# omahs/cess

Hardware: AMD Instinct MI355X
Metric: verified BLS12-381 sigs/sec (node) (higher is better)
Workload: dtype u32 (381-bit Montgomery, 14x28-bit limb products via v_mad_u64_u32)

## Files before the change

cess_amd/csrc/bls/consts.hpp:

```cpp
#pragma once
#include <stdint.h>
#ifndef CESS_CONST
#define CESS_CONST static constexpr
#endif
namespace bls { namespace c {
CESS_CONST uint32_t P_RAW[12] = {0xffffaaabu, 0xb9feffffu, 0xb153ffffu, 0x1eabfffeu, 0xf6b0f624u, 0x6730d2a0u, 0xf38512bfu, 0x64774b84u, 0x434bacd7u, 0x4b1ba7b6u, 0x397fe69au, 0x1a0111eau};
CESS_CONST uint32_t P2_RAW[12] = {0xffff5556u, 0x73fdffffu, 0x62a7ffffu, 0x3d57fffdu, 0xed61ec48u, 0xce61a541u, 0xe70a257eu, 0xc8ee9709u, 0x869759aeu, 0x96374f6cu, 0x72ffcd34u, 0x340223d4u};
CESS_CONST uint32_t ONE[12] = {0x0347fcb8u, 0x19d80000u, 0x6d2002b1u, 0x12e00cdeu, 0xa2090c72u, 0x37669f83u, 0xda0f73e0u, 0x09b09b42u, 0x8f1297bbu, 0xa7c515d9u, 0xfcfa012cu, 0x0577a659u};
CESS_CONST uint32_t R2[12] = {0x510370edu, 0x626d1c34u, 0xc53e243du, 0xd65aec45u, 0x3317d3b1u, 0x4f36a009u, 0x5d74088bu, 0x8c10ea72u, 0x75865d11u, 0xd507320au, 0xa759fd5cu, 0x0c8d4cc8u};
CESS_CONST uint32_t R2_384[12] = {0xc4d1dd0eu, 0x9941d94cu, 0x51c109f3u, 0xff568cb5u, 0x0df0c2b7u, 0x1cc8ea98u, 0x76862c67u, 0xdbf76e0cu, 0x47ae37e1u, 0xcef527bfu, 0x56b3b194u, 0x0834704du};
CESS_CONST uint32_t P28[14] = {0xfffaaabu, 0xfefffffu, 0x3ffffb9u, 0xfffeb15u, 0x6241eabu, 0xa0f6b0fu, 0xf6730d2u, 0xf38512bu, 0x4774b84u, 0x4bacd76u, 0xba7b643u, 0xe69a4b1u, 0x1ea397fu, 0x001a011u};
CESS_CONST uint32_t PINV28 = 0xffcfffdu;
CESS_CONST uint64_t LAZY_M28[27] = {0x00ffffffe3d23e09ull, 0x01ffffffc33e0cc0ull, 0x02ffffffa2fb1340ull, 0x03ffffff81972cd3ull, 0x04ffffff647caecaull, 0x05ffffff4a164486ull, 0x06ffffff2ac97b1dull, 0x07ffffff05982188ull, 0x08fffffee339dc81ull, 0x09fffffec4896d6cull, 0x0afffffea94ef357ull, 0x0bfffffe8fee1d33ull, 0x0cfffffe6bb828c3ull, 0x0c01fffe5fe0053full, 0x0b01fffe7fe0000dull, 0x0a01fffe9fe0000cull, 0x0901fffebfe0000bull, 0x0801fffedfe0000aull, 0x0701fffeffe00009ull, 0x0601ffff1fe00008ull, 0x0501ffff3fe00007ull, 0x0401ffff5fe00006ull, 0x0301ffff7fe00005ull, 0x0201ffff9fe00004ull, 0x0101ffffbfe00003ull, 0x0001ffffdfe00002ull, 0x000000ffffe00001ull};
CESS_CONST uint32_t NEG_K28[14] = {0x1ffcaaaeu, 0x1f5ffffeu, 0x17fffd42u, 0x1fff2ed3u, 0x1d6932b6u, 0x149a2e98u, 0x1a07e839u, 0x18332bb6u, 0x1ca8f330u, 0x1f4c069du, 0x148d1e9fu, 0x10206ef0u, 0x13263efeu, 0x001040aau};
CESS_CONST uint32_t HALF[12] = {0x01a3fe5cu, 0x8cec0000u, 0x36900158u, 0x0970066fu, 0xd1048639u, 0x1bb34fc1u, 0x6d07b9f0u, 0x84d84da1u, 0xc7894bddu, 0x53e28aecu, 0xfe7d0096u, 0x02bbd32cu};
CESS_CONST uint32_t P_HALF_RAW[12] = {0xffffd555u, 0xdcff7fffu, 0x58a9ffffu, 0x0f55ffffu, 0x7b587b12u, 0xb3986950u, 0x79c2895fu, 0xb23ba5c2u, 0x21a5d66bu, 0x258dd3dbu, 0x1cbff34du, 0x0d0088f5u};
CESS_CONST uint32_t EXP_SQRT[12] = {0xffffeaabu, 0xee7fbfffu, 0xac54ffffu, 0x07aaffffu, 0x3dac3d89u, 0xd9cc34a8u, 0x3ce144afu, 0xd91dd2e1u, 0x90d2eb35u, 0x92c6e9edu, 0x8e5ff9a6u, 0x0680447au};
CESS_CONST uint32_t EXP_SQRT_RATIO[12] = {0xffffeaaau, 0xee7fbfffu, 0xac54ffffu, 0x07aaffffu, 0x3dac3d89u, 0xd9cc34a8u, 0x3ce144afu, 0xd91dd2e1u, 0x90d2eb35u, 0x92c6e9edu, 0x8e5ff9a6u, 0x0680447au};
CESS_CONST uint32_t EXP_INV[12] = {0xffffaaa9u, 0xb9feffffu, 0xb153ffffu, 0x1eabfffeu, 0xf6b0f624u, 0x6730d2a0u, 0xf38512bfu, 0x64774b84u, 0x434bacd7u, 0x4b1ba7b6u, 0x397fe69au, 0x1a0111eau};
CESS_CONST uint32_t EXP_LEGENDRE[12] = {0xffffd555u, 0xdcff7fffu, 0x58a9ffffu, 0x0f55ffffu, 0x7b587b12u, 0xb3986950u, 0x79c2895fu, 0xb23ba5c2u, 0x21a5d66bu, 0x258dd3dbu, 0x1cbff34du, 0x0d0088f5u};
CESS_CONST int32_t P30[13] = {1073719979, 670826495, 356515835, 721420204, 821437470, 55215066, 288093811, 316751073, 752313463, 517541166, 698659258, 982409209, 1704209};
CESS_CONST uint32_t PINV30 = 0x00030003u;
CESS_CONST uint32_t R3[12] = {0xd1f7b890u, 0x22294cc4u, 0x56c9f3afu, 0xc0ccb5bau, 0xd975ccb5u, 0x89a8c5c0u, 0x6c968b4cu, 0x922672eau, 0xa691de8cu, 0x7c835652u, 0xbbb98497u, 0x141ab424u};
CESS_CONST uint32_t B1[12] = {0x0d1ff2e0u, 0x67600000u, 0xb4800ac4u, 0x4b803379u, 0x882431c8u, 0xdd9a7e0eu, 0x683dcf80u, 0x26c26d0bu, 0x3c4a5eecu, 0x9f145766u, 0xf3e804b2u, 0x15de9967u};
CESS_CONST uint32_t B1_3[12] = {0x2760834au, 0xc2220000u, 0xbad8204du, 0xa5289a6fu, 0xab0aa910u, 0xca6dd4e9u, 0x51af4903u, 0xab58b018u, 0x2e47c315u, 0x4705b6c6u, 0x68b840e3u, 0x0d99a863u};
CESS_CONST uint32_t ISO_A[12] = {0xf5effb65u, 0x8c7b0e9au, 0xbe82c368u, 0x3be02e2fu, 0x56b8ef09u, 0x1e099c4eu, 0x22aa2e75u, 0xdbb7ea2bu, 0x0b50194eu, 0xe5daee9fu, 0x15b24130u, 0x197623acu};
CESS_CONST uint32_t ISO_B[12] = {0x22b73540u, 0x19a971feu, 0x1f2d700du, 0xfe3eb3afu, 0xed883b92u, 0x7b2b6ba0u, 0x40a0c1b2u, 0x2054e265u, 0x7fed52aeu, 0xabcbf6c9u, 0x2a3ec537u, 0x01fbe6b3u};
CESS_CONST uint32_t ISO_Z[12] = {0x24188692u, 0xa84a0000u, 0x4db81d9cu, 0x92488d91u, 0x09019c9eu, 0x93073566u, 0x779fd523u, 0xa1a814d5u, 0x9f352b5au, 0x9f40a0ecu, 0x6bbe3fb6u, 0x08220209u};
CESS_CONST uint32_t SSWU_C2[12] = {0xb725794eu, 0x7f22ed8fu, 0x1d4f79f9u, 0x8b00a470u, 0xb7dfc3d5u, 0x50a61c22u, 0x3e5e7100u, 0xaa63a15eu, 0x42dee6cfu, 0xe9d7983fu, 0x81ab3cc6u, 0x16957b33u};
CESS_CONST uint32_t ISO_XNUM[12][12] = {
  {0x0030c68du, 0x6f0ff3afu, 0x58ae8c65u, 0x50559808u, 0xbb941b8bu, 0x488cb750u, 0x566f7fb4u, 0xef70f3bau, 0x5ab13d41u, 0x3ebb84a2u, 0x2347c92du, 0x095ee59cu},
  {0xdbd48ae9u, 0x67ca385cu, 0x0dc2aa9cu, 0x35883d22u, 0x4f70e280u, 0xc7b8ce92u, 0xc3459f7eu, 0x23c7c377u, 0xea1ce578u, 0x73b9bab1u, 0x080b857bu, 0x0731f178u},
  {0x0b7ea03du, 0x38a13a48u, 0x5474c6b9u, 0xb25dc086u, 0x803f76afu, 0x36032168u, 0x91fe8ec7u, 0xae8d3767u, 0xf96c2fefu, 0x03b69d83u, 0xfadc62e0u, 0x19c7030cu},
  {0xf756eb7bu, 0x68b02870u, 0x96442170u, 0x79d13078u, 0x1672bf7eu, 0x5111d1abu, 0xe867e73cu, 0x7f5bb8e6u, 0xb90cfcb3u, 0xe66ac958u, 0xe2a91b35u, 0x0d3b3013u},
  {0xa76d9a35u, 0x74d84bd6u, 0x8edd85abu, 0x3af08ac0u, 0xace720cbu, 0x010984b5u, 0x9f144189u, 0x3af083bbu, 0x6ace1173u, 0x1bbf470au, 0x89b595a0u, 0x17a6e3ceu},
  {0x36786159u, 0xdc88e2f4u, 0x1773bdb0u, 0xed909be2u, 0x6c992d13u, 0x708bcf0cu, 0x7065e9e6u, 0xe46986bau, 0xeedc350au, 0x46b5c69fu, 0x2f217806u, 0x11b9a68bu},
  {0x406a5219u, 0x44a5c953u, 0x6debe955u, 0x94636a45u, 0x3ac15bf0u, 0x4388515fu, 0xccc0cdd8u, 0xd70433e1u, 0xde316386u, 0xbe0ad5c7u, 0x7e7af3e8u, 0x153e1c94u},
  {0x06c4fb39u, 0x3345490fu, 0x50198191u, 0xc978a8efu, 0xa2a25687u, 0x96fa653fu, 0xacde2b85u, 0x49e351e0u, 0x8be08e5eu, 0xb04642dcu, 0x0a589780u, 0x15078731u},
  {0xd5d06035u, 0xf8a6ba78u, 0xe7907600u, 0xb78e9a9du, 0x3a2e70d4u, 0x6f4027e9u, 0xca1ab0f2u, 0x04521c42u, 0xd6527145u, 0x312250dfu, 0x162f4b8fu, 0x0c3213dbu},
  {0xf59006e1u, 0x542057bfu, 0xae8cb227u, 0xe938aee4u, 0x158421eau, 0xd9fee33au, 0x265a8059u, 0x54ffe802u, 0x8ac3af4bu, 0xfa85721au, 0xa7ecaef6u, 0x19e875c7u},
  {0xd93b1c44u, 0xe8957e7du, 0x4e6375f4u, 0x3347d486u, 0x5e569fa8u, 0xb9f41161u, 0xff751c3cu, 0x8796563du, 0x6482b424u, 0x103a5579u, 0x6f8744f3u, 0x07a7a82bu},
  {0x8dc7255au, 0x081c5065u, 0xb64bd5b5u, 0xc0f9fbdeu, 0x31629965u, 0xddaf670eu, 0xdc3e32f9u, 0x48aab07bu, 0x9334cba9u, 0x4edd208fu, 0xe5895fd6u, 0x19679604u},
};
CESS_CONST uint32_t ISO_XDEN[11][12] = {
  {0xb0fd9a51u, 0xf0ad77fdu, 0xd8cfa0bcu, 0x1ab81000u, 0x4fc8c4d1u, 0x0fdbda12u, 0x2d514b09u, 0x25b4a5d0u, 0xeeb84fc4u, 0x3ad344e7u, 0xc192a9c6u, 0x139c83aeu},
  {0x06dc8390u, 0x07ea3ba5u, 0xfad76a39u, 0x3a0a0afcu, 0x3ea41449u, 0xea08deeau, 0x5718b76au, 0x089282c4u, 0xe47a41c2u, 0xcc8c2957u, 0x89f9beb5u, 0x132e3dbbu},
  {0xa01ea679u, 0x4457a644u, 0x414ff0c1u, 0x5138cd96u, 0xa3c1ff44u, 0xcb3565d7u, 0xf78713b0u, 0x823832d0u, 0x205c7943u, 0x7f3699d0u, 0x8db2ab31u, 0x0721cf12u},
  {0x792b40c5u, 0xb07d1182u, 0x96f0fc13u, 0x52369016u, 0x4df721dbu, 0x7a63e350u, 0xb6c0e973u, 0x32b09fafu, 0xba296357u, 0x3e594fb7u, 0x45d59b6eu, 0x07942202u},
  {0xcb46256au, 0x8c27ae6au, 0xde781f8du, 0x0697334eu, 0x7ebfc1b5u, 0xc6964917u, 0xb8920defu, 0xb79f25b1u, 0x1912b792u, 0x1d9b36f0u, 0x63d35487u, 0x046cd06eu},
  {0x142f1feau, 0x9dc822cdu, 0x1335b50du, 0x640c4295u, 0x5e5bb0fau, 0x508cdba8u, 0x71eeecb3u, 0x128c7eb1u, 0x2770f8a9u, 0x90b2e7dau, 0xc1c277e7u, 0x17f98f72u},
  {0xb2683982u, 0x7bf01151u, 0xd511b3f5u, 0x0b2c65e2u, 0x35d76bfcu, 0xc6f287d3u, 0x4a5bf52du, 0x8fcfa49bu, 0x473c2339u, 0x6875a07fu, 0x4d7220e1u, 0x0afce898u},
  {0x77164c08u, 0xacf07478u, 0x1b60f0a8u, 0xfda50d29u, 0xc0621366u, 0x0c32f8d9u, 0xcb162619u, 0xb046659fu, 0xd8e78056u, 0x5ad2dbadu, 0xf8b826e8u, 0x00714b65u},
  {0x133e522eu, 0x2875439cu, 0xb527a73cu, 0x41dc3b0fu, 0x403c0cf3u, 0x67751331u, 0x54df788eu, 0x77adcbabu, 0xbd4648eau, 0x242ecadeu, 0xb0c6e99du, 0x13ae78ceu},
  {0xacfc06c3u, 0x80cbc97bu, 0xce86c0cbu, 0x0b6f73a8u, 0xdcbfcf90u, 0xc8af6b03u, 0x7328c888u, 0x59bf7020u, 0x4e6e83d1u, 0x66ca7875u, 0xda730fcau, 0x10190981u},
  {0x0347fcb8u, 0x19d80000u, 0x6d2002b1u, 0x12e00cdeu, 0xa2090c72u, 0x37669f83u, 0xda0f73e0u, 0x09b09b42u, 0x8f1297bbu, 0xa7c515d9u, 0xfcfa012cu, 0x0577a659u},
};
CESS_CONST uint32_t ISO_YNUM[16][12] = {
  {0x839d66d5u, 0x9d00f3e2u, 0xfd53674eu, 0xd8f25861u, 0x6e476ae9u, 0x02f5c6e8u, 0xb6c56d5bu, 0x9185fc0cu, 0x80047b42u, 0xa22923aau, 0x308fdcbdu, 0x157d3dcdu},
  {0x426b9433u, 0xecbc5fa5u, 0x1c2c78b5u, 0x281fcccfu, 0x562d8276u, 0x6bbbccccu, 0x30bf3d5bu, 0x7438cf87u, 0x6a63196bu, 0x2b062c40u, 0x1ecf8d5cu, 0x173fa485u},
  {0x5d378f14u, 0x7206922au, 0x61ce7d49u, 0x0283e46eu, 0x768c198eu, 0x04413947u, 0x486e9644u, 0x15674c1du, 0x062f8917u, 0x4f9aeba4u, 0xb93c7762u, 0x0e3a3c37u},
  {0xafe4102fu, 0xca7095bfu, 0xab5b077bu, 0xdc15a6f4u, 0x648cdaeeu, 0x28e016a7u, 0x19a5e73eu, 0xc0090a40u, 0xde2d52edu, 0x8922ee6fu, 0xb72dc063u, 0x0852d865u},
  {0x8a5c944au, 0x5784c7ffu, 0x3da6fd62u, 0x3874e39fu, 0xf5274f65u, 0x3ab6d533u, 0x1990e200u, 0x87ac98edu, 0xa8149cd2u, 0xf122067bu, 0x788bece6u, 0x11fcdb49u},
  {0x1bc3324fu, 0x631d3111u, 0xeb4d82aau, 0x03fcf5f2u, 0xd4b0a4f3u, 0x04fd2761u, 0x2c0443c5u, 0xf9e5fa4au, 0x1df333adu, 0xc8118fa7u, 0x4399765bu, 0x0fcb068bu},
  {0xa7f2fa91u, 0xb3bfb0d7u, 0xf0f6197au, 0x227181e7u, 0x5443b505u, 0xf33c8d61u, 0x5b830d30u, 0x7af1b579u, 0x30dbfe3cu, 0x7b44aa16u, 0x9465c351u, 0x18c8c64eu},
  {0xc4f07932u, 0xdcff72f7u, 0x0c8891b0u, 0x9b5a9101u, 0x8a0bca41u, 0xaf0f47c2u, 0x201a4c44u, 0xe4434f2du, 0x06f7d374u, 0xe11e0f0bu, 0x9a64fe11u, 0x10ba38eau},
  {0x0da2a912u, 0x50f3844eu, 0x7f6a33c8u, 0x0b99a459u, 0xabcc2e50u, 0xebf8233du, 0x8033b735u, 0x40b10cc1u, 0xd39ed605u, 0xcb035820u, 0xff879de9u, 0x17c40f98u},
  {0x12e219b0u, 0xccaeb03cu, 0xe88a1787u, 0xd9b5fb43u, 0xf1052bffu, 0x97c94700u, 0x02ecb329u, 0x6f222476u, 0x25ea5876u, 0x96f42a4cu, 0xa9f29adau, 0x01bc972cu},
// ... 68 lines not shown
```

cess_amd/csrc/bls/curve.hpp:

```cpp
#pragma once
#include "field.hpp"

namespace bls {

template <class F>
struct proj {
  F x, y, z;
};
template <class F>
struct affine {
  F x, y;
  bool inf;
};
using g1p = proj<fp>;
using g2p = proj<fp2>;
using g1a = affine<fp>;
using g2a = affine<fp2>;

CESS_HD fp mul_b3(const fp& a) { return mul4(mul3(a)); }
CESS_HD fp2 mul_b3(const fp2& a) { return mul4(mul3(mul_nr(a))); }
template <class F> CESS_HD F f_zero();
template <> CESS_HD fp f_zero<fp>() { return fp_zero(); }
template <> CESS_HD fp2 f_zero<fp2>() { return fp2_zero(); }
template <class F> CESS_HD F f_one();
template <> CESS_HD fp f_one<fp>() { return fp_one(); }
template <> CESS_HD fp2 f_one<fp2>() { return fp2_one(); }

template <class F>
CESS_HD proj<F> proj_identity() {
  return {f_zero<F>(), f_one<F>(), f_zero<F>()};
}
template <class F>
CESS_HD proj<F> proj_from_affine(const affine<F>& a) {
  if (a.inf) return proj_identity<F>();
  return {a.x, a.y, f_one<F>()};
}

template <class F>
CESS_HD proj<F> proj_dbl(const proj<F>& p) {
  F t0 = sqr(p.y);
  F z3 = mul8(t0);
  F t1 = mul(p.y, p.z);
  F t2 = sqr(p.z);
  t2 = mul_b3(t2);
  F x3 = mul(t2, z3);
  F y3 = add(t0, t2);
  z3 = mul(t1, z3);
  t1 = dbl(t2);
  t2 = add(t1, t2);
  t0 = sub(t0, t2);
  y3 = mul(t0, y3);
  y3 = add(x3, y3);
  t1 = mul(p.x, p.y);
  x3 = mul(t0, t1);
// ... 195 lines not shown
CESS_HD g1p g1_mul_glv(const fp& px, const fp& py, const uint32_t (&k)[8]) {
  uint32_t k1[4], k2[4];
  glv_split(k, k1, k2);
  const g1p P2 = proj_dbl(g1p{px, py, fp_one()});
  const g1p P3 = proj_add_mixed(P2, px, py);
  const fp zi = inv(mul(P2.z, P3.z));
  const fp z2i = mul(zi, P3.z), z3i = mul(zi, P2.z);
  const fp x2 = mul(P2.x, z2i), y2 = mul(P2.y, z2i), x3 = mul(P3.x, z3i), y3 = mul(P3.y, z3i);
  const fp beta = fp_from(c::G1_BETA);
  const fp beta2 = mul(beta, beta);
  g1p acc = proj_identity<fp>();
#pragma unroll 1
  for (int w = 63; w >= 0; w--) {
    acc = proj_dbl(proj_dbl(acc));
    const int sh = 2 * (w & 15);
    const uint32_t d1 = (k1[w >> 4] >> sh) & 3u, d2 = (k2[w >> 4] >> sh) & 3u;
    {
      const fp tx = select(d1 == 1, px, select(d1 == 2, x2, x3)), ty = select(d1 == 1, py, select(d1 == 2, y2, y3));
      const g1p s = proj_add_mixed(acc, tx, ty);
      acc = {select(d1 != 0, s.x, acc.x), select(d1 != 0, s.y, acc.y), select(d1 != 0, s.z, acc.z)};
    }
    {
      const fp tx = mul(select(d2 == 1, px, select(d2 == 2, x2, x3)), beta2);
      const fp ty = select(d2 == 1, py, select(d2 == 2, y2, y3));
      const g1p s = proj_add_mixed(acc, tx, ty);
      acc = {select(d2 != 0, s.x, acc.x), select(d2 != 0, s.y, acc.y), select(d2 != 0, s.z, acc.z)};
    }
  }
  return acc;
}

CESS_HD g1p jac_dbl(const g1p& p) {
  const fp A = sqr(p.x), B = sqr(p.y), C = sqr(B);
  const fp D = dbl(sub(sub(sqr(add(p.x, B)), A), C));
  const fp E = mul3(A);
  const fp x3 = sub(sqr(E), dbl(D));
  const fp y3 = sub(mul(E, sub(D, x3)), mul8(C));
  const fp z3 = dbl(mul(p.y, p.z));
  return {x3, y3, z3};
}
CESS_HD g1p jac_add_mixed(const g1p& p, const fp& qx, const fp& qy) {
  const fp z1z1 = sqr(p.z);
  const fp u2 = mul(qx, z1z1), s2 = mul(qy, mul(p.z, z1z1));
  const fp h = sub(u2, p.x), hh = sqr(h);
  const fp i = mul4(hh), j = mul(h, i);
  const fp r = dbl(sub(s2, p.y));
  const fp v = mul(p.x, i);
  const fp x3 = sub(sub(sqr(r), j), dbl(v));
  const fp y3 = sub(mul(r, sub(v, x3)), dbl(mul(p.y, j)));
  const fp z3 = sub(sub(sqr(add(p.z, h)), z1z1), hh);
  return {x3, y3, z3};
}

CESS_HD g1p g1_mul_glv32(const fp& px, const fp& py, uint32_t a, uint32_t b) {
  const g1p P2 = proj_dbl(g1p{px, py, fp_one()});
  const g1p P3 = proj_add_mixed(P2, px, py);
  const fp zi = inv(mul(P2.z, P3.z));
  const fp z2i = mul(zi, P3.z), z3i = mul(zi, P2.z);
  const fp x2 = mul(P2.x, z2i), y2 = mul(P2.y, z2i), x3 = mul(P3.x, z3i), y3 = mul(P3.y, z3i);
  const fp beta = fp_from(c::G1_BETA);
  g1p acc = {fp_zero(), fp_one(), fp_zero()};
  bool id = true;
#pragma unroll 1
  for (int bp = 30; bp >= 0; bp -= 2) {
    acc = jac_dbl(jac_dbl(acc));
#pragma unroll 1
    for (int h = 0; h < 2; h++) {
      const uint32_t d = ((h ? b : a) >> bp) & 3u;
      fp tx = select(d == 1, px, select(d == 2, x2, x3));
      const fp ty = select(d == 1, py, select(d == 2, y2, y3));
      if (h) tx = mul(tx, beta);
      const g1p sum = jac_add_mixed(acc, tx, ty);
      const bool take = d != 0;
      acc = {select(take, select(id, tx, sum.x), acc.x), select(take, select(id, ty, sum.y), acc.y),
             select(take, select(id, fp_one(), sum.z), acc.z)};
      id = id && !take;
    }
  }
  if (id) return proj_identity<fp>();
  return {mul(acc.x, acc.z), acc.y, mul(sqr(acc.z), acc.z)};
}

CESS_HD bool g1_is_torsion_free(const fp& px, const fp& py) {
  constexpr uint64_t X2_HI = 0xac45a4010001a402ull, X2_LO = 0x0000000100000000ull;
  g1p acc = {px, py, fp_one()};
#pragma unroll 1
  for (int b = 126; b >= 0; b--) {
    acc = jac_dbl(acc);
    const uint64_t w = b >= 64 ? X2_HI : X2_LO;
    if ((w >> (b & 63)) & 1u) acc = jac_add_mixed(acc, px, py);
  }
  const fp z2 = sqr(acc.z), z3 = mul(z2, acc.z);
  return !is_zero(acc.z) && eq(mul(mul(px, fp_from(c::G1_BETA)), z2), acc.x) && eq(mul(py, z3), neg(acc.y));
}
CESS_HD bool g1_is_torsion_free_rcb(const fp& px, const fp& py) {
  g1p xp = proj_mul_u64_mixed(px, py, BLS_X_ABS);
  g1p x2p = proj_mul_u64(xp, BLS_X_ABS);
  g1p phi = {mul(px, fp_from(c::G1_BETA)), py, fp_one()};
  return proj_eq(phi, proj_neg(x2p));
}
CESS_HD fp2 psi_x_coeff() { return {fp_from(c::PSI_X_C0), fp_from(c::PSI_X_C1)}; }
CESS_HD fp2 psi_y_coeff() { return {fp_from(c::PSI_Y_C0), fp_from(c::PSI_Y_C1)}; }
template <class Park>
CESS_HD bool g2_is_torsion_free(const fp2& px, const fp2& py, const Park& pk) {
  pk.st(0, px);
  pk.st(1, py);
  g2p xp = proj_mul_u64_mixed_ld<fp2>([&](fp2& x, fp2& y) { x = pk.ld(0), y = pk.ld(1); }, BLS_X_ABS);
  CESS_MEMBAR();
  g2p psi = {mul(conj(pk.ld(0)), psi_x_coeff()), mul(conj(pk.ld(1)), psi_y_coeff()), fp2_one()};
  return proj_eq(psi, proj_neg(xp));
}
struct RegPark2 {
  fp2 v[2];
  CESS_HD fp2 ld(int k) const { return v[k]; }
  CESS_HD void st(int k, const fp2& a) const { const_cast<RegPark2*>(this)->v[k] = a; }
};

CESS_HD fp raw_from_be_words(const uint32_t* w) {
  fp r;
#pragma unroll
  for (int i = 0; i < 12; i++) r.v[i] = w[11 - i];
  return r;
}

CESS_HD bool g1_decompress(const uint32_t* w, g1a& out) {
  uint32_t flags = w[0] >> 29;
  bool cflag = flags & 4, iflag = flags & 2, sflag = flags & 1;
  fp xr = raw_from_be_words(w);
  xr.v[11] &= 0x1fffffffu;
  out.inf = false;
  out.x = fp_zero();
  out.y = fp_one();
  if (!raw_lt_p(xr)) return false;
  if (iflag && cflag && !sflag && is_zero(xr)) {
    out.inf = true;
    return true;
  }
  if (iflag || !cflag) return false;
  fp x = to_mont(xr);
  fp y;
  if (!sqrt(y, add(mul(sqr(x), x), fp_from(c::B1)))) return false;
  if (lex_largest(y) != sflag) y = neg(y);
  if (!g1_is_torsion_free(x, y)) return false;
  out.x = x;
  out.y = y;
  return true;
// ... 65 lines not shown
```

cess_amd/csrc/bls/h2c.hpp:

```cpp
#pragma once
#include "curve.hpp"

namespace bls {

CESS_CONST uint32_t SHA_K[64] = {
    0x428a2f98u, 0x71374491u, 0xb5c0fbcfu, 0xe9b5dba5u, 0x3956c25bu, 0x59f111f1u, 0x923f82a4u, 0xab1c5ed5u,
    0xd807aa98u, 0x12835b01u, 0x243185beu, 0x550c7dc3u, 0x72be5d74u, 0x80deb1feu, 0x9bdc06a7u, 0xc19bf174u,
    0xe49b69c1u, 0xefbe4786u, 0x0fc19dc6u, 0x240ca1ccu, 0x2de92c6fu, 0x4a7484aau, 0x5cb0a9dcu, 0x76f988dau,
    0x983e5152u, 0xa831c66du, 0xb00327c8u, 0xbf597fc7u, 0xc6e00bf3u, 0xd5a79147u, 0x06ca6351u, 0x14292967u,
    0x27b70a85u, 0x2e1b2138u, 0x4d2c6dfcu, 0x53380d13u, 0x650a7354u, 0x766a0abbu, 0x81c2c92eu, 0x92722c85u,
    0xa2bfe8a1u, 0xa81a664bu, 0xc24b8b70u, 0xc76c51a3u, 0xd192e819u, 0xd6990624u, 0xf40e3585u, 0x106aa070u,
    0x19a4c116u, 0x1e376c08u, 0x2748774cu, 0x34b0bcb5u, 0x391c0cb3u, 0x4ed8aa4au, 0x5b9cca4fu, 0x682e6ff3u,
    0x748f82eeu, 0x78a5636fu, 0x84c87814u, 0x8cc70208u, 0x90befffau, 0xa4506cebu, 0xbef9a3f7u, 0xc67178f2u};
CESS_CONST uint32_t SHA_IV[8] = {0x6a09e667u, 0xbb67ae85u, 0x3c6ef372u, 0xa54ff53au,
                                 0x510e527fu, 0x9b05688cu, 0x1f83d9abu, 0x5be0cd19u};

CESS_HD uint32_t rotr32(uint32_t x, int n) { return (x >> n) | (x << (32 - n)); }

CESS_HD void sha256_compress(uint32_t (&st)[8], const uint32_t (&blk)[16]) {
  uint32_t w[16];
#pragma unroll
  for (int i = 0; i < 16; i++) w[i] = blk[i];
  uint32_t a = st[0], b = st[1], cc = st[2], d = st[3], e = st[4], f = st[5], g = st[6], h = st[7];
#pragma unroll
// ... 139 lines not shown
  fp y2 = mul(y1, fp_from(c::SSWU_C2));
  bool is_qr = eq(mul(sqr(y1), gxd), gxn);
  fp yy = select(is_qr, y1, y2);
  fp x = mul(tv1, tv3);
  fp ycand = mul(mul(tv1, u), yy);
  xn = select(is_qr, tv3, x);
  y = select(is_qr, yy, ycand);
  if (sgn0(u) != sgn0(y)) y = neg(y);
  xd = tv4;
}

CESS_HD g1p iso_map_proj(const fp& X, const fp& Y, const fp& Z) {
  fp aXN = fp_zero(), aXD = fp_zero(), aYN = fp_zero(), aYD = fp_zero(), D = fp_one();
#pragma unroll 1
  for (int i = 15; i >= 0; i--) {
    if (i < 15) {
      D = mul(D, Z);
      aYN = mul(aYN, X);
      aYD = mul(aYD, X);
      if (i < 11) aXN = mul(aXN, X);
      if (i < 10) aXD = mul(aXD, X);
    }
    aYN = add(aYN, mul(fp_from(c::ISO_YNUM[i]), D));
    aYD = add(aYD, mul(fp_from(c::ISO_YDEN[i]), D));
    if (i <= 11) aXN = add(aXN, mul(fp_from(c::ISO_XNUM[i]), D));
    if (i <= 10) aXD = add(aXD, mul(fp_from(c::ISO_XDEN[i]), D));
  }
  const fp yd = mul(aYD, Z);
  return {mul(aXN, yd), mul(mul(Y, aYN), aXD), mul(aXD, yd)};
}

CESS_HD g1p iso_curve_add(const g1p& p, const g1p& q) {
  const fp A = fp_from(c::ISO_A), B3 = mul3(fp_from(c::ISO_B));
  fp t0 = mul(p.x, q.x), t1 = mul(p.y, q.y), t2 = mul(p.z, q.z);
  fp t3 = sub(mul(add_nr(p.x, p.y), add_nr(q.x, q.y)), add(t0, t1));
  fp t4 = sub(mul(add_nr(p.x, p.z), add_nr(q.x, q.z)), add(t0, t2));
  fp t5 = sub(mul(add_nr(p.y, p.z), add_nr(q.y, q.z)), add(t1, t2));
  fp z3 = add(mul(B3, t2), mul(A, t4));
  fp x3 = sub(t1, z3);
  z3 = add(t1, z3);
  fp y3 = mul(x3, z3);
  t1 = add(dbl(t0), t0);
  t2 = mul(A, t2);
  t4 = mul(B3, t4);
  t1 = add(t1, t2);
  t2 = mul(A, sub(t0, t2));
  t4 = add(t4, t2);
  y3 = add(y3, mul(t1, t4));
  x3 = sub(mul(t3, x3), mul(t5, t4));
  z3 = add(mul(t5, z3), mul(t3, t1));
  return {x3, y3, z3};
}

CESS_HD g1a clear_cofactor_g1(const fp& rx, const fp& ry) {
  g1p acc = {rx, ry, fp_one()};
#pragma unroll 1
  for (int b = 62; b >= 0; b--) {
    acc = jac_dbl(acc);
    if ((H_EFF_G1 >> b) & 1u) acc = jac_add_mixed(acc, rx, ry);
  }
  if (is_zero(acc.z)) return proj_to_affine(proj_mul_u64_mixed(rx, ry, H_EFF_G1));
  const fp iz = inv(acc.z), iz2 = sqr(iz);
  g1a r;
  r.inf = false;
  r.x = mul(acc.x, iz2);
  r.y = mul(acc.y, mul(iz2, iz));
  return r;
}

CESS_HD g1a hash_to_g1(const uint8_t* msg, uint32_t len) {
  uint32_t uni[32];
  expand_message_xmd_128(msg, len, uni);
  g1p s;
#pragma unroll 1
  for (int j = 0; j < 2; j++) {
    uint32_t w[16];
#pragma unroll
    for (int k = 0; k < 16; k++) w[k] = j ? uni[16 + k] : uni[k];
    fp xn, xd, y;
    map_to_curve_sswu(fp_from_be64_words(w), xn, xd, y);
    const g1p q = {xn, mul(y, xd), xd};
    s = j ? iso_curve_add(s, q) : q;
  }
  g1a r;
  r.inf = true;
  r.x = fp_zero();
  r.y = fp_one();
  if (is_zero(s.z)) return r;
  const g1p t = iso_map_proj(s.x, s.y, s.z);
  if (is_zero(t.z)) return r;
  const fp zi = inv(t.z);
  return clear_cofactor_g1(mul(t.x, zi), mul(t.y, zi));
}

#if !defined(CESS_HOSTEMU)
CESS_HD void park_fp(uint32_t (*park)[256], int row, uint32_t t, const fp& a) {
#pragma unroll
  for (int i = 0; i < 12; i++) park[row + i][t] = a.v[i];
}
CESS_HD fp unpark_fp(uint32_t (*park)[256], int row, uint32_t t) {
  fp a;
#pragma unroll
  for (int i = 0; i < 12; i++) a.v[i] = park[row + i][t];
  return a;
}
CESS_HD g1a hash_to_g1_parked(const uint8_t* msg, uint32_t len, uint32_t (*park)[256], uint32_t t) {
  fp u0;
  {
    uint32_t uni[32];
    expand_message_xmd_128<true>(msg, len, uni);
    uint32_t w[16];
#pragma unroll
    for (int k = 0; k < 16; k++) w[k] = uni[16 + k];
// ... 36 lines not shown
```

cess_amd/csrc/gen_consts.py:

```python
import hashlib
import os
import struct

BLS_X = 0xd201000000010000
X = -BLS_X
R = X**4 - X**2 + 1
P = (X - 1) ** 2 * R // 3 + X
RM = 1 << 392

ISO_A = 0x144698a3b8e9433d693a02c96d4982b0ea985383ee66a8d8e8981aefd881ac98936f8da0e0f97f5cf428082d584c1d
ISO_B = 0x12e2908d11688030018b12e8753eee3b2016c1f0f24f4070a0b9c14fcef35ef55a23215a316ceaa5d1cc48e98e172be0
ISO_Z = 11
ISO_XNUM = [
    0x11a05f2b1e833340b809101dd99815856b303e88a2d7005ff2627b56cdb4e2c85610c2d5f2e62d6eaeac1662734649b7,
    0x17294ed3e943ab2f0588bab22147a81c7c17e75b2f6a8417f565e33c70d1e86b4838f2a6f318c356e834eef1b3cb83bb,
    0x0d54005db97678ec1d1048c5d10a9a1bce032473295983e56878e501ec68e25c958c3e3d2a09729fe0179f9dac9edcb0,
    0x1778e7166fcc6db74e0609d307e55412d7f5e4656a8dbf25f1b33289f1b330835336e25ce3107193c5b388641d9b6861,
    0x0e99726a3199f4436642b4b3e4118e5499db995a1257fb3f086eeb65982fac18985a286f301e77c451154ce9ac8895d9,
    0x1630c3250d7313ff01d1201bf7a74ab5db3cb17dd952799b9ed3ab9097e68f90a0870d2dcae73d19cd13c1c66f652983,
    0x0d6ed6553fe44d296a3726c38ae652bfb11586264f0f8ce19008e218f9c86b2a8da25128c1052ecaddd7f225a139ed84,
    0x17b81e7701abdbe2e8743884d1117e53356de5ab275b4db1a682c62ef0f2753339b7c8f8c8f475af9ccb5618e3f0c88e,
    0x080d3cf1f9a78fc47b90b33563be990dc43b756ce79f5574a2c596c928c5d1de4fa295f296b74e956d71986a8497e317,
    0x169b1f8e1bcfa7c42e0c37515d138f22dd2ecb803a0c5c99676314baf4bb1b7fa3190b2edc0327797f241067be390c9e,
    0x10321da079ce07e272d8ec09d2565b0dfa7dccdde6787f96d50af36003b14866f69b771f8c285decca67df3f1605fb7b,
# ... 144 lines not shown
    a, b, c, d, e, f, g, h = state
    for i in range(64):
        S1 = rotr(e, 6) ^ rotr(e, 11) ^ rotr(e, 25)
        ch = (e & f) ^ (~e & g)
        t1 = (h + S1 + ch + k[i] + w[i]) & M
        S0 = rotr(a, 2) ^ rotr(a, 13) ^ rotr(a, 22)
        maj = (a & b) ^ (a & c) ^ (b & c)
        t2 = (S0 + maj) & M
        h, g, f, e, d, c, b, a = g, f, e, (d + t1) & M, c, b, a, (t1 + t2) & M
    return [(x + y) & M for x, y in zip(state, (a, b, c, d, e, f, g, h))]


SHA_IV = [0x6a09e667, 0xbb67ae85, 0x3c6ef372, 0xa54ff53a, 0x510e527f, 0x9b05688c, 0x1f83d9ab, 0x5be0cd19]


def main():
    out = []
    w = out.append
    w("// GENERATED by cess_amd/csrc/gen_consts.py — do not edit.")
    w("// BLS12-381 constants, 12 x u32 little-endian limbs; MONT = Montgomery form (R = 2^392).")
    w("#pragma once")
    w("#include <stdint.h>")
    w("#ifndef CESS_CONST")
    w("#define CESS_CONST static constexpr")
    w("#endif")
    w("namespace bls { namespace c {")

    def arr(name, v, n=12):
        w(f"CESS_CONST uint32_t {name}[{n}] = {{" + ", ".join(f"0x{x:08x}u" for x in limbs(v, n)) + "};")

    arr("P_RAW", P)
    arr("P2_RAW", 2 * P)
    arr("ONE", mont(1))
    arr("R2", RM * RM % P)
    arr("R2_384", (1 << 384) * RM * RM % P)
    p28 = [(P >> (28 * i)) & 0xFFFFFFF for i in range(14)]
    w("CESS_CONST uint32_t P28[14] = {" + ", ".join(f"0x{x:07x}u" for x in p28) + "};")
    w(f"CESS_CONST uint32_t PINV28 = 0x{(-pow(P, -1, 1 << 28)) % (1 << 28):07x}u;")
    L = [(1 << 28) - 1] * 13 + [(1 << 20) - 1]
    B = [sum(L[i] * L[k - i] for i in range(14) if 0 <= k - i < 14) for k in range(27)]
    D = sum(b << (28 * k) for k, b in enumerate(B))
    adj = (-D) % P
    for k in range(14):
        B[k] += (adj >> (28 * k)) & ((1 << 28) - 1)
    M = sum(b << (28 * k) for k, b in enumerate(B))
    assert M % P == 0 and M < (1 << 770) and max(B) < (1 << 60)
    w("CESS_CONST uint64_t LAZY_M28[27] = {" + ", ".join(f"0x{x:016x}ull" for x in B) + "};")
    base = [(1 << 28) - 1] * 13 + [(1 << 20) - 1]
    bv = sum(b << (28 * k) for k, b in enumerate(base))
    adj = (-bv) % P
    K = [base[k] + ((adj >> (28 * k)) & ((1 << 28) - 1)) for k in range(14)]
    assert sum(k << (28 * i) for i, k in enumerate(K)) % P == 0 and max(K) < (1 << 29)
    w("CESS_CONST uint32_t NEG_K28[14] = {" + ", ".join(f"0x{x:08x}u" for x in K) + "};")
    arr("HALF", mont((P + 1) // 2))
    arr("P_HALF_RAW", (P - 1) // 2)
    arr("EXP_SQRT", (P + 1) // 4)
    arr("EXP_SQRT_RATIO", (P - 3) // 4)
    arr("EXP_INV", P - 2)
    arr("EXP_LEGENDRE", (P - 1) // 2)
    w("CESS_CONST int32_t P30[13] = {" + ", ".join(str((P >> (30 * i)) & ((1 << 30) - 1)) for i in range(13)) + "};")
    w(f"CESS_CONST uint32_t PINV30 = 0x{pow(P, -1, 1 << 30):08x}u;")
    arr("R3", RM ** 3 % P)
    arr("B1", mont(4))
    arr("B1_3", mont(12))
    arr("ISO_A", mont(ISO_A))
    arr("ISO_B", mont(ISO_B))
    arr("ISO_Z", mont(ISO_Z))
    c2 = pow((-ISO_Z) % P, (P + 1) // 4, P)
    assert c2 * c2 % P == (-ISO_Z) % P
    arr("SSWU_C2", mont(c2))
    for name, lst in (("ISO_XNUM", ISO_XNUM), ("ISO_XDEN", ISO_XDEN), ("ISO_YNUM", ISO_YNUM), ("ISO_YDEN", ISO_YDEN)):
        w(f"CESS_CONST uint32_t {name}[{len(lst)}][12] = {{")
        for v in lst:
            w("  {" + ", ".join(f"0x{x:08x}u" for x in limbs(mont(v))) + "},")
        w("};")
    beta = None
    for cand in range(2, 40):
        b = pow(cand, (P - 1) // 3, P)
        if b == 1:
            continue
        for bb in (b, b * b % P):
            phi = (G1_GEN[0] * bb % P, G1_GEN[1])
            if phi == smul(G1_GEN, -(X * X), FP_OPS):
                beta = bb
        if beta:
            break
    assert beta
    arr("G1_BETA", mont(beta))
    xi = (1, 1)
    psi_x = f2inv(f2pow(xi, (P - 1) // 3))
    psi_y = f2inv(f2pow(xi, (P - 1) // 2))
    gx, gy = G2_GEN
    psi_g = (f2mul((gx[0], -gx[1] % P), psi_x), f2mul((gy[0], -gy[1] % P), psi_y))
    assert psi_g == smul(G2_GEN, X, FP2_OPS), "psi constant check"
    for name, v in (("PSI_X", psi_x), ("PSI_Y", psi_y)):
        arr(name + "_C0", mont(v[0]))
        arr(name + "_C1", mont(v[1]))
    w("CESS_CONST uint32_t FROB[3][6][2][12] = {")
    for k in (1, 2, 3):
        w("  {")
        for i in range(6):
            g = f2pow(xi, i * (P ** k - 1) // 6)
            w("    {{" + ", ".join(f"0x{x:08x}u" for x in limbs(mont(g[0]))) + "}, {" +
              ", ".join(f"0x{x:08x}u" for x in limbs(mont(g[1]))) + "}},")
        w("  },")
    w("};")
# ... 22 lines not shown
```

Before: 3.218 million.

## Add bound-typed lazy 28-bit digit field arithmetic for G1 scalar loops

Introduces a 14-digit 28-bit field representation whose digit and value bounds are tracked in the type. This lets add, sub, neg and scale skip carries and modular reductions, and lets mul and sqr accept unreduced inputs. Jacobian doubling and mixed addition are rewritten on this type and used in the G1 torsion check and the G1 cofactor clearing. The goal is to cut per-operation pack and unpack work and the reductions in these long double-and-add chains. The risk is the correctness of the bound tracking and the extra conversions at the loop boundaries.

```diff
diff --git a/cess_amd/csrc/bls/consts.hpp b/cess_amd/csrc/bls/consts.hpp
--- a/cess_amd/csrc/bls/consts.hpp
+++ b/cess_amd/csrc/bls/consts.hpp
@@ -13,6 +13,16 @@
 CESS_CONST uint32_t PINV28 = 0xffcfffdu;
 CESS_CONST uint64_t LAZY_M28[27] = {0x00ffffffe3d23e09ull, 0x01ffffffc33e0cc0ull, 0x02ffffffa2fb1340ull, 0x03ffffff81972cd3ull, 0x04ffffff647caecaull, 0x05ffffff4a164486ull, 0x06ffffff2ac97b1dull, 0x07ffffff05982188ull, 0x08fffffee339dc81ull, 0x09fffffec4896d6cull, 0x0afffffea94ef357ull, 0x0bfffffe8fee1d33ull, 0x0cfffffe6bb828c3ull, 0x0c01fffe5fe0053full, 0x0b01fffe7fe0000dull, 0x0a01fffe9fe0000cull, 0x0901fffebfe0000bull, 0x0801fffedfe0000aull, 0x0701fffeffe00009ull, 0x0601ffff1fe00008ull, 0x0501ffff3fe00007ull, 0x0401ffff5fe00006ull, 0x0301ffff7fe00005ull, 0x0201ffff9fe00004ull, 0x0101ffffbfe00003ull, 0x0001ffffdfe00002ull, 0x000000ffffe00001ull};
 CESS_CONST uint32_t NEG_K28[14] = {0x1ffcaaaeu, 0x1f5ffffeu, 0x17fffd42u, 0x1fff2ed3u, 0x1d6932b6u, 0x149a2e98u, 0x1a07e839u, 0x18332bb6u, 0x1ca8f330u, 0x1f4c069du, 0x148d1e9fu, 0x10206ef0u, 0x13263efeu, 0x001040aau};
+CESS_CONST int DD_VV_MAX = 2515;
+CESS_CONST uint32_t DD_NEG_P28[14] = {0x0005555u, 0x0100000u, 0xc000046u, 0x00014eau, 0x9dbe154u, 0x5f094f0u, 0x098cf2du, 0x0c7aed4u, 0xb88b47bu, 0xb453289u, 0x45849bcu, 0x1965b4eu, 0xe15c680u, 0xffe5feeu};
+CESS_CONST uint32_t DD_K_D1_V2[14] = {0x1fff0001u, 0x1fcffffeu, 0x1bffff2cu, 0x1fffc13eu, 0x126c5c02u, 0x1e2e412du, 0x1e359276u, 0x1da8f382u, 0x1d65e28du, 0x1e306861u, 0x12f722c8u, 0x1b3cee14u, 0x15beac7eu, 0x0004e032u};
+CESS_CONST uint32_t DD_K_D2_V4[14] = {0x2ffe5557u, 0x2faffffdu, 0x23fffe9fu, 0x2fff9768u, 0x2eb49959u, 0x224d174au, 0x2d03f41bu, 0x2c1995d9u, 0x26547996u, 0x27a6034du, 0x2a468f4eu, 0x28103776u, 0x29931f7du, 0x00082053u};
+CESS_CONST uint32_t DD_K_D3_V6[14] = {0x3ffdaaadu, 0x3f8ffffcu, 0x3bfffe12u, 0x3fff6d91u, 0x3afcd6b0u, 0x366bed68u, 0x3bd255bfu, 0x3a8a3830u, 0x3f43109fu, 0x311b9e38u, 0x3195fbd4u, 0x34e380d9u, 0x3d67927cu, 0x000b6074u};
+CESS_CONST uint32_t DD_K_D4_V8[14] = {0x4ffd0003u, 0x4f6ffffbu, 0x43fffd85u, 0x4fff43bbu, 0x47451407u, 0x4a8ac386u, 0x4aa0b763u, 0x48fada87u, 0x4831a7a8u, 0x4a913924u, 0x48e56859u, 0x41b6ca3bu, 0x413c057bu, 0x000ea096u};
+CESS_CONST uint32_t DD_K_D9_V18[14] = {0x9ff9aab1u, 0x9ecffff6u, 0x9bfffac4u, 0x9ffe728au, 0x94ae46bau, 0x9f24f21bu, 0x94a89f98u, 0x912e063au, 0x94da9ad5u, 0x99dd3fbeu, 0x9d7286f5u, 0x91d73927u, 0x94624475u, 0x001ee13cu};
+CESS_CONST uint32_t DD_K_D1_V9[14] = {0x1ffcaaaeu, 0x1f5ffffeu, 0x17fffd42u, 0x1fff2ed3u, 0x1d6932b6u, 0x149a2e98u, 0x1a07e839u, 0x18332bb6u, 0x1ca8f330u, 0x1f4c069du, 0x148d1e9fu, 0x10206ef0u, 0x13263efeu, 0x001040aau};
+CESS_CONST uint32_t DD_K_D1_V27[14] = {0x1ff6aab4u, 0x1e3ffffeu, 0x1ffff856u, 0x1ffdb651u, 0x1bf35aceu, 0x19afb5adu, 0x1f495708u, 0x1a28e0cdu, 0x1d0c4289u, 0x146e78eeu, 0x1657ef5bu, 0x138e036fu, 0x159e49fcu, 0x002d81deu};
+CESS_CONST uint32_t DD_K_D4_V19[14] = {0x4ff9555cu, 0x4ebffffbu, 0x4ffffa83u, 0x4ffe5da4u, 0x4ad2656bu, 0x49345d2fu, 0x440fd070u, 0x4066576bu, 0x4951e65fu, 0x4e980d39u, 0x491a3d3du, 0x4040dddeu, 0x464c7dfau, 0x00208152u};
 CESS_CONST uint32_t HALF[12] = {0x01a3fe5cu, 0x8cec0000u, 0x36900158u, 0x0970066fu, 0xd1048639u, 0x1bb34fc1u, 0x6d07b9f0u, 0x84d84da1u, 0xc7894bddu, 0x53e28aecu, 0xfe7d0096u, 0x02bbd32cu};
 CESS_CONST uint32_t P_HALF_RAW[12] = {0xffffd555u, 0xdcff7fffu, 0x58a9ffffu, 0x0f55ffffu, 0x7b587b12u, 0xb3986950u, 0x79c2895fu, 0xb23ba5c2u, 0x21a5d66bu, 0x258dd3dbu, 0x1cbff34du, 0x0d0088f5u};
 CESS_CONST uint32_t EXP_SQRT[12] = {0xffffeaabu, 0xee7fbfffu, 0xac54ffffu, 0x07aaffffu, 0x3dac3d89u, 0xd9cc34a8u, 0x3ce144afu, 0xd91dd2e1u, 0x90d2eb35u, 0x92c6e9edu, 0x8e5ff9a6u, 0x0680447au};
diff --git a/cess_amd/csrc/bls/curve.hpp b/cess_amd/csrc/bls/curve.hpp
--- a/cess_amd/csrc/bls/curve.hpp
+++ b/cess_amd/csrc/bls/curve.hpp
@@ -1,5 +1,6 @@
 #pragma once
 #include "field.hpp"
+#include "field_d.hpp"
 
 namespace bls {
 
@@ -301,6 +302,42 @@
   return {x3, y3, z3};
 }
 
+struct g1jd {
+  fd<1, 27> x;
+  fd<4, 19> y;
+  fd<1, 7> z;
+};
+CESS_HD g1jd g1jd_from_affine(const fd<1, 2>& x, const fd<1, 2>& y) {
+  return {widen<1, 27>(x), widen<4, 19>(y), widen<1, 7>(from_fp(fp_one()))};
+}
+CESS_HD g1jd jac_dbl_d(const g1jd& p) {
+  const auto A = sqr(p.x), B = sqr(p.y);
+  const auto z3 = mul(scale<2>(p.y), p.z);
+  const auto C = sqr(B);
+  const auto S = sqr(add(p.x, B));
+  const auto AC = add(A, C);
+  const auto Mn = sub(AC, S);
+  const auto EE = sqr(scale<3>(A));
+  const auto x3 = normalise(add(add(EE, scale<4>(AC)), neg(scale<4>(S))));
+  const auto W = normalise(add(scale<2>(Mn), x3));
+  const auto y3 = normalise(neg(add(mul(scale<3>(A), W), scale<8>(C))));
+  return {x3, widen<4, 19>(y3), widen<1, 7>(z3)};
+}
+CESS_HD g1jd jac_add_mixed_d(const g1jd& p, const fd<1, 2>& qx, const fd<1, 2>& qy) {
+  const auto z1z1 = sqr(p.z);
+  const auto u2 = mul(qx, z1z1), s2 = mul(qy, mul(p.z, z1z1));
+  const auto h = sub(u2, p.x);
+  const auto hh = sqr(h);
+  const auto i = scale<4>(hh);
+  const auto j = mul(h, i);
+  const auto r = scale<2>(normalise(sub(s2, p.y)));
+  const auto v = mul(p.x, i);
+  const auto x3 = normalise(sub(sqr(r), add(j, scale<2>(v))));
+  const auto y3 = sub(mul(r, sub(v, x3)), mul(scale<2>(p.y), j));
+  const auto z3 = normalise(sub(sqr(add(p.z, h)), add(z1z1, hh)));
+  return {widen<1, 27>(x3), widen<4, 19>(y3), z3};
+}
+
 CESS_HD g1p g1_mul_glv32(const fp& px, const fp& py, uint32_t a, uint32_t b) {
   const g1p P2 = proj_dbl(g1p{px, py, fp_one()});
   const g1p P3 = proj_add_mixed(P2, px, py);
@@ -330,8 +367,24 @@
   return {mul(acc.x, acc.z), acc.y, mul(sqr(acc.z), acc.z)};
 }
 
+#ifndef CESS_DIGIT_G1
+#define CESS_DIGIT_G1 1
+#endif
 CESS_HD bool g1_is_torsion_free(const fp& px, const fp& py) {
   constexpr uint64_t X2_HI = 0xac45a4010001a402ull, X2_LO = 0x0000000100000000ull;
+#if CESS_DIGIT_G1
+  const fd<1, 2> qx = from_fp(px), qy = from_fp(py);
+  g1jd acc = g1jd_from_affine(qx, qy);
+#pragma unroll 1
+  for (int b = 126; b >= 0; b--) {
+    acc = jac_dbl_d(acc);
+    const uint64_t w = b >= 64 ? X2_HI : X2_LO;
+    if ((w >> (b & 63)) & 1u) acc = jac_add_mixed_d(acc, qx, qy);
+  }
+  const auto z2 = sqr(acc.z), z3 = mul(z2, acc.z);
+  const fp bx = to_fp(mul(mul(qx, from_fp(fp_from(c::G1_BETA))), z2)), yz = to_fp(mul(qy, z3));
+  return !is_zero(to_fp(acc.z)) && eq(bx, to_fp(acc.x)) && eq(yz, neg(to_fp(acc.y)));
+#else
   g1p acc = {px, py, fp_one()};
 #pragma unroll 1
   for (int b = 126; b >= 0; b--) {
@@ -341,6 +394,7 @@
   }
   const fp z2 = sqr(acc.z), z3 = mul(z2, acc.z);
   return !is_zero(acc.z) && eq(mul(mul(px, fp_from(c::G1_BETA)), z2), acc.x) && eq(mul(py, z3), neg(acc.y));
+#endif
 }
 CESS_HD bool g1_is_torsion_free_rcb(const fp& px, const fp& py) {
   g1p xp = proj_mul_u64_mixed(px, py, BLS_X_ABS);
diff --git a/cess_amd/csrc/bls/field_d.hpp b/cess_amd/csrc/bls/field_d.hpp
--- /dev/null
+++ b/cess_amd/csrc/bls/field_d.hpp
@@ -0,0 +1,217 @@
+#pragma once
+#include "field.hpp"
+
+#if defined(CESS_DIGIT_CHECK)
+#if !defined(CESS_HOSTEMU)
+#error "CESS_DIGIT_CHECK is a host-emulation mode"
+#endif
+#include <stdio.h>
+#endif
+
+namespace bls {
+
+template <int D, int V>
+struct fd {
+  static_assert(D >= 1 && D <= 16 && V >= 1, "digits are 32-bit words");
+  uint32_t d[14];
+};
+
+#if defined(CESS_DIGIT_CHECK)
+namespace dchk {
+inline uint64_t g_fail = 0, g_checked = 0;
+inline void fail(const char* op, const char* what) {
+  if (g_fail++ < 16) fprintf(stderr, "digit check: %s: %s\n", op, what);
+}
+inline bool value_ok(const uint32_t (&d)[14], int V) {
+  uint64_t l[18] = {0}, r[18] = {0};
+  for (int i = 0; i < 14; i++) l[i] = (uint64_t)d[i] * 1024u, r[i] = (uint64_t)c::P28[i] * 1025u * (uint64_t)V;
+  for (int i = 0; i < 17; i++) {
+    l[i + 1] += l[i] >> 28, l[i] &= M28;
+    r[i + 1] += r[i] >> 28, r[i] &= M28;
+  }
+  for (int i = 17; i >= 0; i--)
+    if (l[i] != r[i]) return l[i] < r[i];
+  return false;
+}
+template <int D, int V>
+inline void val(const fd<D, V>& x, const char* op) {
+  g_checked++;
+  for (int i = 0; i < 14; i++)
+    if ((uint64_t)x.d[i] >= ((uint64_t)D << 28)) return fail(op, "digit above its bound");
+  if (!value_ok(x.d, V)) fail(op, "value above its bound");
+}
+inline void columns(const uint32_t (&x)[14], const uint32_t (&y)[14], const char* op) {
+  unsigned __int128 acc = 0;
+  uint32_t m[14];
+  for (int k = 0; k < 27; k++) {
+    for (int i = 0; i < 14; i++)
+      if (k - i >= 0 && k - i < 14) acc += (unsigned __int128)x[i] * y[k - i];
+    for (int i = k < 14 ? 0 : k - 13; i < (k < 14 ? k : 14); i++) acc += (unsigned __int128)m[i] * c::P28[k - i];
+    if (k < 14) {
+      m[k] = ((uint32_t)acc * c::PINV28) & M28;
+      acc += (unsigned __int128)m[k] * c::P28[0];
+    }
+    if (acc >> 64) return fail(op, "column sum above 2^64");
+    acc >>= 28;
+  }
+}
+}
+#define CESS_DCHK_VAL(x, op) dchk::val(x, op)
+#define CESS_DCHK_COLS(x, y, op) dchk::columns(x, y, op)
+#else
+#define CESS_DCHK_VAL(x, op) ((void)0)
+#define CESS_DCHK_COLS(x, y, op) ((void)0)
+#endif
+
+template <int D, int V>
+struct dd_k;
+#define CESS_DD_K(D, V)                                                      \
+  template <>                                                                \
+  struct dd_k<D, V> {                                                        \
+    static CESS_HD uint32_t at(int i) { return c::DD_K_D##D##_V##V[i]; }     \
+  };
+CESS_DD_K(1, 2)
+CESS_DD_K(2, 4)
+CESS_DD_K(3, 6)
+CESS_DD_K(4, 8)
+CESS_DD_K(9, 18)
+CESS_DD_K(1, 9)
+CESS_DD_K(1, 27)
+CESS_DD_K(4, 19)
+#undef CESS_DD_K
+
+CESS_HD fd<1, 2> from_fp(const fp& a) {
+  fd<1, 2> r;
+  unpack28(a, r.d);
+  CESS_DCHK_VAL(r, "from_fp");
+  return r;
+}
+
+template <int D2, int V2, int D, int V>
+CESS_HD fd<D2, V2> widen(const fd<D, V>& a) {
+  static_assert(D2 >= D && V2 >= V, "widen only loosens");
+  fd<D2, V2> r;
+#pragma unroll
+  for (int i = 0; i < 14; i++) r.d[i] = a.d[i];
+  return r;
+}
+
+template <int Da, int Va, int Db, int Vb>
+CESS_HD fd<Da + Db, Va + Vb> add(const fd<Da, Va>& a, const fd<Db, Vb>& b) {
+  CESS_DCHK_VAL(a, "add");
+  CESS_DCHK_VAL(b, "add");
+  fd<Da + Db, Va + Vb> r;
+#pragma unroll
+  for (int i = 0; i < 14; i++) r.d[i] = a.d[i] + b.d[i];
+  CESS_DCHK_VAL(r, "add result");
+  return r;
+}
+
+template <int S, int D, int V>
+CESS_HD fd<S * D, S * V> scale(const fd<D, V>& a) {
+  static_assert(S >= 2 && S <= 12, "small multiples");
+  CESS_DCHK_VAL(a, "scale");
+  fd<S * D, S * V> r;
+#pragma unroll
+  for (int i = 0; i < 14; i++) r.d[i] = a.d[i] * (uint32_t)S;
+  CESS_DCHK_VAL(r, "scale result");
+  return r;
+}
+
+template <int D, int V>
+CESS_HD fd<D + 1, V + 1> neg(const fd<D, V>& b) {
+  CESS_DCHK_VAL(b, "neg");
+  fd<D + 1, V + 1> r;
+#pragma unroll
+  for (int i = 0; i < 14; i++) r.d[i] = dd_k<D, V>::at(i) - b.d[i];
+  CESS_DCHK_VAL(r, "neg result");
+  return r;
+}
+
+template <int Da, int Va, int Db, int Vb>
+CESS_HD fd<Da + Db + 1, Va + Vb + 1> sub(const fd<Da, Va>& a, const fd<Db, Vb>& b) {
+  CESS_DCHK_VAL(a, "sub");
+  CESS_DCHK_VAL(b, "sub");
+  fd<Da + Db + 1, Va + Vb + 1> r;
+#pragma unroll
+  for (int i = 0; i < 14; i++) r.d[i] = a.d[i] + (dd_k<Db, Vb>::at(i) - b.d[i]);
+  CESS_DCHK_VAL(r, "sub result");
+  return r;
+}
+
+template <int D, int V>
+CESS_HD fd<1, V> normalise(const fd<D, V>& a) {
+  static_assert(D <= 15, "digit + carry must fit 32 bits");
+  static_assert(V <= 1024, "the value must fit 14 digits");
+  CESS_DCHK_VAL(a, "normalise");
+  fd<1, V> r;
+  uint32_t cy = 0;
+#pragma unroll
+  for (int i = 0; i < 13; i++) {
+    const uint32_t s = a.d[i] + cy;
+    r.d[i] = s & M28V;
+    cy = s >> 28;
+  }
+  r.d[13] = a.d[13] + cy;
+  CESS_DCHK_VAL(r, "normalise result");
+  return r;
+}
+
+template <int V>
+CESS_HD fd<1, 2> reduce_small(const fd<1, V>& a) {
+  static_assert(V <= 64, "q (2^392 - p) digit sums stay far below 2^64; remainder < 2p");
+  CESS_DCHK_VAL(a, "reduce_small");
+  const uint32_t q = a.d[13] / (c::P28[13] + 1u);
+  fd<1, 2> r;
+  uint64_t acc = 0;
+#pragma unroll
+  for (int i = 0; i < 14; i++) {
+    acc += a.d[i];
+    mac(acc, q, c::DD_NEG_P28[i]);
+    r.d[i] = (uint32_t)acc & M28V;
+    acc >>= 28;
+  }
+  CESS_DCHK_VAL(r, "reduce_small result");
+  return r;
+}
+
+template <int Da, int Va, int Db, int Vb>
+CESS_HD fd<1, 2> mul(const fd<Da, Va>& a, const fd<Db, Vb>& b) {
+  static_assert(Da * Db <= 16, "column sums: 14 Da Db 2^56 + 14 2^56 + carry < 2^64");
+  static_assert(Va * Vb <= c::DD_VV_MAX, "double-width value below p R");
+  CESS_DCHK_VAL(a, "mul");
+  CESS_DCHK_VAL(b, "mul");
+  CESS_DCHK_COLS(a.d, b.d, "mul");
+  fd<1, 2> r;
+  mul_d(r.d, a.d, b.d);
+  CESS_DCHK_VAL(r, "mul result");
+  return r;
+}
+template <int D, int V>
+CESS_HD fd<1, 2> sqr(const fd<D, V>& a) {
+  static_assert(D * D <= 16, "column sums (the doubled digits also fit 32 bits)");
+  static_assert(V * V <= c::DD_VV_MAX, "double-width value below p R");
+  CESS_DCHK_VAL(a, "sqr");
+  CESS_DCHK_COLS(a.d, a.d, "sqr");
+  fd<1, 2> r;
+#pragma unroll
+  for (int i = 0; i < 14; i++) r.d[i] = a.d[i];
+  sqr_d(r.d);
+  CESS_DCHK_VAL(r, "sqr result");
+  return r;
+}
+
+CESS_HD fp to_fp(const fd<1, 2>& a) {
+  CESS_DCHK_VAL(a, "to_fp");
+  return pack28(a.d);
+}
+template <int V>
+CESS_HD fp to_fp(const fd<1, V>& a) {
+  return to_fp(reduce_small(a));
+}
+template <int D, int V>
+CESS_HD fp to_fp(const fd<D, V>& a) {
+  return to_fp(reduce_small(normalise(a)));
+}
+
+}
diff --git a/cess_amd/csrc/bls/h2c.hpp b/cess_amd/csrc/bls/h2c.hpp
--- a/cess_amd/csrc/bls/h2c.hpp
+++ b/cess_amd/csrc/bls/h2c.hpp
@@ -215,13 +215,30 @@
   return {x3, y3, z3};
 }
 
+#ifndef CESS_DIGIT_H2C
+#define CESS_DIGIT_H2C 1
+#endif
 CESS_HD g1a clear_cofactor_g1(const fp& rx, const fp& ry) {
+#if CESS_DIGIT_H2C
+  g1p acc;
+  {
+    const fd<1, 2> qx = from_fp(rx), qy = from_fp(ry);
+    g1jd t = g1jd_from_affine(qx, qy);
+#pragma unroll 1
+    for (int b = 62; b >= 0; b--) {
+      t = jac_dbl_d(t);
+      if ((H_EFF_G1 >> b) & 1u) t = jac_add_mixed_d(t, qx, qy);
+    }
+    acc = {to_fp(t.x), to_fp(t.y), to_fp(t.z)};
+  }
+#else
   g1p acc = {rx, ry, fp_one()};
 #pragma unroll 1
   for (int b = 62; b >= 0; b--) {
     acc = jac_dbl(acc);
     if ((H_EFF_G1 >> b) & 1u) acc = jac_add_mixed(acc, rx, ry);
   }
+#endif
   if (is_zero(acc.z)) return proj_to_affine(proj_mul_u64_mixed(rx, ry, H_EFF_G1));
   const fp iz = inv(acc.z), iz2 = sqr(iz);
   g1a r;
diff --git a/cess_amd/csrc/gen_consts.py b/cess_amd/csrc/gen_consts.py
--- a/cess_amd/csrc/gen_consts.py
+++ b/cess_amd/csrc/gen_consts.py
@@ -220,6 +220,19 @@
     K = [base[k] + ((adj >> (28 * k)) & ((1 << 28) - 1)) for k in range(14)]
     assert sum(k << (28 * i) for i, k in enumerate(K)) % P == 0 and max(K) < (1 << 29)
     w("CESS_CONST uint32_t NEG_K28[14] = {" + ", ".join(f"0x{x:08x}u" for x in K) + "};")
+    un, ud = 1025, 1024
+    w(f"CESS_CONST int DD_VV_MAX = {(RM * ud * ud) // (P * un * un)};")
+    np28 = [((RM - P) >> (28 * i)) & 0xFFFFFFF for i in range(14)]
+    w("CESS_CONST uint32_t DD_NEG_P28[14] = {" + ", ".join(f"0x{x:07x}u" for x in np28) + "};")
+    for D, V in ((1, 2), (2, 4), (3, 6), (4, 8), (9, 18), (1, 9), (1, 27), (4, 19)):
+        top = (V * P * un // ud) >> 364
+        base = [D * (1 << 28) - 1] * 13 + [top]
+        bv = sum(b << (28 * k) for k, b in enumerate(base))
+        adj = (-bv) % P
+        K = [base[k] + ((adj >> (28 * k)) & ((1 << 28) - 1)) for k in range(13)] + [top + (adj >> 364)]
+        kv = sum(k << (28 * i) for i, k in enumerate(K))
+        assert kv % P == 0 and max(K) < ((D + 1) << 28) <= (1 << 32) and kv * ud < (V + 1) * P * un
+        w(f"CESS_CONST uint32_t DD_K_D{D}_V{V}[14] = {{" + ", ".join(f"0x{x:08x}u" for x in K) + "};")
     arr("HALF", mont((P + 1) // 2))
     arr("P_HALF_RAW", (P - 1) // 2)
     arr("EXP_SQRT", (P + 1) // 4)
```

Result: no change. 3.249 million, median of 6 (+1.0%).
